# belinghy/SteppingStone

Measured on AMD Instinct MI355X. Metric: env-steps/sec (batched random-action rollout), higher is better.
Workload: dtype f32; 1 GPU; Walker3DStepperEnv-v0, 4096 envs per MI355X, curriculum 0 (flat terrain), on-device Philox U(-1,1) actions, auto-reset on; envs_total=4096, parallelism=env-shard x1, ranks=1, steps_per_launch=1000, prewarm_steps=256

## Files before the change

steppingstone_amd/csrc/ss_kernels.hpp:

```cpp
#pragma once
#include <cstdlib>

#include "ss_dynamics.hpp"
#include "../../include/steppingstone.h"

namespace ss {

enum { F_POS = 0, F_QUAT = 3, F_VEL = 7, F_Q = 13, F_QD = 34, F_POT = 55, F_ZINIT = 56, F_EPRET = 57, F_NNDR = 58,
       F_STONE = 59, F_HEAD = 59 + 24, F_EPRET_LO = 59 + 30, NF = 59 + 30 + 1 };
enum { I_N = 0, I_COUNT = 1, I_ELAPSED = 2, I_RNG = 3, I_FLAGS = 4, I_PROV = 5, NI = 6 };
constexpr int kNumStones = 20;
constexpr int kNumSubsteps = 4;
constexpr float kDeg = 0.017453292519943295f;

struct Knobs {
  const float* prob;
  int per_env_prob;
  int curriculum;
  float power;
  int auto_reset;
};

struct Params {
  float* fstate;
// ... 48 lines not shown
  philox4x32_10(ctr, 0u, P.env_offset + ((uint32_t)e & P.id_mask), 0u, P.seed_lo, P.seed_hi, out);
  ctr += 1u;
}

SSD int sample_cell(const Params& P, const Knobs& K, int e, float u) {
  float cdf = 0.f;
  int last = 0, pick = -1;
  const float* pr = K.per_env_prob ? K.prob + e : K.prob;
  const int stride = K.per_env_prob ? P.npad : 1;
#pragma unroll 1
  for (int k = 0; k < SS_NCELL; ++k) {
    float pk = pr[(size_t)k * stride];
    if (pk > 0.f) last = k;
    cdf += pk;
    if (pick < 0 && u < cdf) pick = k;
  }
  return pick < 0 ? last : pick;
}

SSD void place_stone(float px, float py, float pz, float dr, float cp, float sp, float cph, float sph, float out_p[3]) {
  float planar = dr * cp;
  out_p[0] = px + planar * cph;
  out_p[1] = py + planar * sph;
  out_p[2] = pz + dr * sp;
}
SSD float draw_stone(const Params& P, const Knobs& K, int e, uint32_t& ctr, int k, float out_p[3], float out_n[3],
                     float out_t[2], float out_h[2], bool store = true) {
  uint32_t r[4];
  env_block(P, e, ctr, r);
  int cell = sample_cell(P, K, e, u01(r[0]));
  float ratio = (float)K.curriculum / 5.0f;
  float dr = 0.65f + u01(r[1]) * (0.6f * ratio);
  float tilt = 15.0f * kDeg * ratio;
  float xt = (2.f * u01(r[2]) - 1.f) * tilt, yt = (2.f * u01(r[3]) - 1.f) * tilt;
  float yaw = yaw_sample(cell / SS_GRID), pitch = pitch_sample(cell % SS_GRID);
  const size_t np = (size_t)P.npad;
  float* T = P.terrain + e;
  int prov = P.istate[e + I_PROV * np];
  const bool prev_stored = k - 1 < prov;
  float px = prev_stored ? T[((k - 1) * 6 + 0) * np] : 0.75f * (float)(k - 1);
  float py = prev_stored ? T[((k - 1) * 6 + 1) * np] : 0.f, pz = prev_stored ? T[((k - 1) * 6 + 2) * np] : 0.f;
  float phi = (prev_stored ? T[((k - 1) * 6 + 3) * np] : 0.f) + yaw;
  float sp, cp, sph, cph;
  sincosf(pitch, &sp, &cp);
  sincosf(phi, &sph, &cph);
  place_stone(px, py, pz, dr, cp, sp, cph, sph, out_p);
  out_t[0] = xt; out_t[1] = yt;
  out_h[0] = cph; out_h[1] = sph;
  stone_normal(phi, xt, yt, out_n);
  if (store) {
#pragma unroll 1
    for (int j = prov; j < k; ++j) {
      T[(j * 6 + 0) * np] = 0.75f * (float)j;
#pragma unroll
      for (int i = 1; i < 6; ++i) T[(j * 6 + i) * np] = 0.f;
    }
    T[(k * 6 + 0) * np] = out_p[0]; T[(k * 6 + 1) * np] = out_p[1]; T[(k * 6 + 2) * np] = out_p[2];
    T[(k * 6 + 3) * np] = phi; T[(k * 6 + 4) * np] = xt; T[(k * 6 + 5) * np] = yt;
    if (prov < k + 1) P.istate[e + I_PROV * np] = k + 1;
  }
  return dr;
}

SSD float planar_dist(const float a[3], const float b[3]) {
  float dx = a[0] - b[0], dy = a[1] - b[1];
  return sqrtf(dx * dx + dy * dy);
}

SSD void quat_roll_pitch_cs(const float q[4], float& roll, float& pitch, float& cy, float& sy) {
  float w = q[0], x = q[1], y = q[2], z = q[3];
  roll = atan2f(2.f * (w * x + y * z), 1.f - 2.f * (x * x + y * y));
  pitch = asinf(fminf(fmaxf(2.f * (w * y - z * x), -1.f), 1.f));
  float A = 1.f - 2.f * (y * y + z * z), B = 2.f * (w * z + x * y);
  float n2 = A * A + B * B;
  float inv = SS_RSQRT(fmaxf(n2, 1e-30f));
  cy = n2 > 1e-30f ? A * inv : 1.f;
  sy = n2 > 1e-30f ? B * inv : 0.f;
}

SSD void target_features(const float pos[3], float cy, float sy, const float sp[3], const float tilt[2], float o[5]) {
  float dx = sp[0] - pos[0], dy = sp[1] - pos[1], dz = sp[2] - pos[2];
  o[0] = dy * cy - dx * sy; o[1] = dx * cy + dy * sy; o[2] = dz; o[3] = tilt[0]; o[4] = tilt[1];
}

SSD float clip5(float x) { return fminf(fmaxf(x, -5.f), 5.f); }
SSD float obs_angle(float ps, float q, float mid, float span) { return clip5(2.f * (ps * q - ps * mid) / span); }
SSD float obs_rate(float ps, float qd) { return clip5(0.1f * (ps * qd)); }

template <class Model>
SSD void write_obs(const Dyn& s, float z_init, int flags, const Cache& c, float* obs) {
  float roll, pitch, sy, cy;
  quat_roll_pitch_cs(s.quat, roll, pitch, cy, sy);
  float R[3][3];
  quat_rot(s.quat, R);
  float vw[3];
#pragma unroll
  for (int r = 0; r < 3; ++r) vw[r] = R[r][0] * s.v0.v[0] + R[r][1] * s.v0.v[1] + R[r][2] * s.v0.v[2];
  obs[0] = clip5(s.pos[2] - z_init);
  obs[1] = clip5(cy * vw[0] + sy * vw[1]);
  obs[2] = clip5(-sy * vw[0] + cy * vw[1]);
  obs[3] = clip5(vw[2]);
  obs[4] = clip5(roll);
  obs[5] = clip5(pitch);
  static_for<0, NJ>([&](auto Jc) {
    constexpr int j = decltype(Jc)::value;
    constexpr float mid = 0.5f * (Model::lo[j] + Model::hi[j]);
    constexpr float span = Model::hi[j] - Model::lo[j];
    constexpr float ps = (float)kPolicySign[j];
    obs[6 + j] = obs_angle(ps, s.q[j], mid, span);
    obs[27 + j] = obs_rate(ps, s.qd[j]);
  });
  obs[48] = (flags & 1) ? 1.f : 0.f;
  obs[49] = (flags & 2) ? 1.f : 0.f;
  float t[5];
  target_features(s.pos, cy, sy, c.p[1], c.tilt[1], t);
#pragma unroll
  for (int i = 0; i < 5; ++i) obs[50 + i] = t[i];
  target_features(s.pos, cy, sy, c.p[2], c.tilt[2], t);
#pragma unroll
  for (int i = 0; i < 5; ++i) obs[55 + i] = t[i];
}

SSD void load_dyn(const Params& P, int e, Dyn& s) {
  const float* F = P.fstate + e;
  const size_t np = (size_t)P.npad;
#pragma unroll
  for (int i = 0; i < 3; ++i) s.pos[i] = F[(F_POS + i) * np];
#pragma unroll
  for (int i = 0; i < 4; ++i) s.quat[i] = F[(F_QUAT + i) * np];
#pragma unroll
  for (int i = 0; i < 3; ++i) { s.v0.w[i] = F[(F_VEL + i) * np]; s.v0.v[i] = F[(F_VEL + 3 + i) * np]; }
#pragma unroll
  for (int j = 0; j < NJ; ++j) { s.q[j] = F[(F_Q + j) * np]; s.qd[j] = F[(F_QD + j) * np]; }
}
SSD void store_dyn(const Params& P, int e, const Dyn& s) {
  float* F = P.fstate + e;
  const size_t np = (size_t)P.npad;
#pragma unroll
  for (int i = 0; i < 3; ++i) F[(F_POS + i) * np] = s.pos[i];
#pragma unroll
  for (int i = 0; i < 4; ++i) F[(F_QUAT + i) * np] = s.quat[i];
#pragma unroll
  for (int i = 0; i < 3; ++i) { F[(F_VEL + i) * np] = s.v0.w[i]; F[(F_VEL + 3 + i) * np] = s.v0.v[i]; }
#pragma unroll
  for (int j = 0; j < NJ; ++j) { F[(F_Q + j) * np] = s.q[j]; F[(F_QD + j) * np] = s.qd[j]; }
}
SSD void load_cache(const Params& P, int e, Cache& c) {
  const float* F = P.fstate + e;
  const size_t np = (size_t)P.npad;
#pragma unroll
  for (int sl = 0; sl < 3; ++sl) {
#pragma unroll
    for (int i = 0; i < 3; ++i) { c.p[sl][i] = F[(F_STONE + sl * 8 + i) * np]; c.nrm[sl][i] = F[(F_STONE + sl * 8 + 3 + i) * np]; }
    c.tilt[sl][0] = F[(F_STONE + sl * 8 + 6) * np];
    c.tilt[sl][1] = F[(F_STONE + sl * 8 + 7) * np];
  }
}
SSD void store_cache(const Params& P, int e, const Cache& c) {
  float* F = P.fstate + e;
  const size_t np = (size_t)P.npad;
#pragma unroll
  for (int sl = 0; sl < 3; ++sl) {
#pragma unroll
    for (int i = 0; i < 3; ++i) { F[(F_STONE + sl * 8 + i) * np] = c.p[sl][i]; F[(F_STONE + sl * 8 + 3 + i) * np] = c.nrm[sl][i]; }
    F[(F_STONE + sl * 8 + 6) * np] = c.tilt[sl][0];
    F[(F_STONE + sl * 8 + 7) * np] = c.tilt[sl][1];
  }
}
SSD void store_headings(const Params& P, int e, const float (&h)[3][2]) {
  float* F = P.fstate + e;
  const size_t np = (size_t)P.npad;
#pragma unroll
  for (int sl = 0; sl < 3; ++sl) { F[(F_HEAD + sl * 2) * np] = h[sl][0]; F[(F_HEAD + sl * 2 + 1) * np] = h[sl][1]; }
}
SSD void cache_from_terrain(const Params& P, int e, int n, Cache& c, float (&hd)[3][2]) {
  const size_t np = (size_t)P.npad;
  const float* T = P.terrain + e;
  int idx[3] = {n - 1 < 0 ? 0 : n - 1, n, n + 1 > kNumStones - 1 ? kNumStones - 1 : n + 1};
#pragma unroll
  for (int sl = 0; sl < 3; ++sl) {
    int k = idx[sl];
#pragma unroll
    for (int i = 0; i < 3; ++i) c.p[sl][i] = T[(k * 6 + i) * np];
    float phi = T[(k * 6 + 3) * np], xt = T[(k * 6 + 4) * np], yt = T[(k * 6 + 5) * np];
    c.tilt[sl][0] = xt; c.tilt[sl][1] = yt;
    stone_normal(phi, xt, yt, c.nrm[sl]);
    sincosf(phi, &hd[sl][1], &hd[sl][0]);
  }
}

SSD void flat_path(Stones& c) {
#pragma unroll
  for (int sl = 0; sl < 3; ++sl) {
    c.p[sl][0] = 0.75f * (float)sl; c.p[sl][1] = 0.f; c.p[sl][2] = 0.f;
    c.nrm[sl][0] = 0.f; c.nrm[sl][1] = 0.f; c.nrm[sl][2] = 1.f;
    c.tilt[sl][0] = 0.f; c.tilt[sl][1] = 0.f;
  }
}
template <class Model, int GJ>
SSD float reset_angle(const uint32_t (&r)[6][4]) {
  constexpr float q0 = Model::q0[GJ], lo = Model::lo[GJ] + 0.02f, hi = Model::hi[GJ] - 0.02f;
  float q = q0 + 0.05f * (2.f * u01(r[GJ / 4][GJ % 4]) - 1.f);
  return fminf(fmaxf(q, lo), hi);
}

template <class Model>
SSD void env_reset(const Params& P, int e, Dyn& s, Cache& c, uint32_t& ctr, float& pot, float& z_init, float& nn_dr) {
  const size_t np = (size_t)P.npad;
  P.istate[e + I_PROV * np] = 0;
  flat_path(c);
  s.pos[0] = 0.f; s.pos[1] = 0.f; s.pos[2] = Model::stand_height + 0.01f;
  s.quat[0] = 1.f; s.quat[1] = s.quat[2] = s.quat[3] = 0.f;
#pragma unroll
  for (int i = 0; i < 3; ++i) { s.v0.w[i] = 0.f; s.v0.v[i] = 0.f; }
  uint32_t r[6][4];
#pragma unroll
  for (int b = 0; b < 6; ++b) env_block(P, e, ctr, r[b]);
  static_for<0, NJ>([&](auto Jc) {
    constexpr int j = decltype(Jc)::value;
    s.q[j] = reset_angle<Model, j>(r);
    s.qd[j] = 0.f;
  });
  z_init = s.pos[2];
  nn_dr = 0.75f;
  pot = -planar_dist(c.p[1], s.pos) / kDt;
}

constexpr int kMaxPeers = 8;
struct PeerTable {
  float* dst[kMaxPeers];
  uint32_t* flag[kMaxPeers];
  uint32_t* done_counter;
  int count;
  int rank;
  int n_local;
};

struct StepIO {
  const float* act;
  float* obs;
  float* rew;
  uint8_t* done;
  ss_info* info;
  uint64_t t;
  float* packed;
  int nsteps;
  const PeerTable* peers;
  uint32_t flag_value;
  long long packed_step_stride;
};

SSD void put_base(const Lds& L, float m, const float pos[3], const float quat[4], const float w[3], const float v[3]) {
  L.s(S_POS + 0) = pos[0]; L.s(S_POS + 1) = m * pos[1]; L.s(S_POS + 2) = pos[2];
  L.s(S_QUAT + 0) = quat[0]; L.s(S_QUAT + 1) = m * quat[1]; L.s(S_QUAT + 2) = quat[2]; L.s(S_QUAT + 3) = m * quat[3];
  L.s(S_VW + 0) = m * w[0]; L.s(S_VW + 1) = w[1]; L.s(S_VW + 2) = m * w[2];
  L.s(S_VV + 0) = v[0]; L.s(S_VV + 1) = m * v[1]; L.s(S_VV + 2) = v[2];
}
SSD void get_base(const Lds& L, float m, float pos[3], float quat[4], SV& v0) {
  pos[0] = L.s(S_POS); pos[1] = m * L.s(S_POS + 1); pos[2] = L.s(S_POS + 2);
  quat[0] = L.s(S_QUAT); quat[1] = m * L.s(S_QUAT + 1); quat[2] = L.s(S_QUAT + 2); quat[3] = m * L.s(S_QUAT + 3);
  v0 = SV{{m * L.s(S_VW), L.s(S_VW + 1), m * L.s(S_VW + 2)}, {L.s(S_VV), m * L.s(S_VV + 1), L.s(S_VV + 2)}};
}
SSD void put_joints(const Lds& L, float m, const float (&q)[NH], const float (&qd)[NH]) {
  static_for<0, NH>([&](auto Kc) {
    constexpr int k = decltype(Kc)::value, jr = kHalf[k];
    const float sg = mirror_sign(jr, m);
    L.s(S_Q + k) = sg * q[k];
    L.s(S_QD + k) = sg * qd[k];
  });
}
SSD void get_joints(const Lds& L, float m, float (&q)[NH], float (&qd)[NH]) {
  static_for<0, NH>([&](auto Kc) {
    constexpr int k = decltype(Kc)::value, jr = kHalf[k];
    const float sg = mirror_sign(jr, m);
    q[k] = sg * L.s(S_Q + k);
    qd[k] = sg * L.s(S_QD + k);
  });
}

struct StepOut {
  float pos[3], quat[4];
  SV v0;
  float qt[NH], qdt[NH];
  float r, z_init, roll, pitch, cyaw, syaw;
  int d, flags, do_reset;
// ... 115 lines not shown
    if constexpr (!ROLLOUT) {
      if (io.peers) {
        constexpr int kPack = SS_OBS_DIM + 2;
        const PeerTable* T = io.peers;
        const int G = T->count;
        const size_t row0 = (size_t)T->rank * (size_t)T->n_local + (size_t)env0;
#pragma unroll 1
        for (int p = 0; p < G; ++p) copy_block(T->dst[p] + row0 * kPack, nvalid * kPack);
        __threadfence_system();
        if (lane == 0) {
          const uint32_t prev = atomicAdd(T->done_counter, 1u);
          if ((prev + 1u) % gridDim.x == 0u) {
            __threadfence_system();
            for (int p = 0; p < G; ++p)
              __hip_atomic_store(T->flag[p] + T->rank, io.flag_value, __ATOMIC_RELEASE, __HIP_MEMORY_SCOPE_SYSTEM);
          }
        }
      }
    }
#endif
  }
#undef SS_OBS
}

constexpr bool out_offload(int helpers, bool rollout) { return rollout && helpers >= 3; }
constexpr int kHandOut = kHandDet, kHandOut2 = kHandFloats;
static_assert(kHandOut2 + 2 <= kHandSlots * 4, "hand-off region");
#if !defined(SS_HOST_HARNESS)
template <class Model, bool ROLLOUT>
__device__ __forceinline__ void emit_from_handoff(const Params& P, const StepIO& io, const Lds& L, int lane, int lane_global, int kstep,
                                                  float* lds) {
  const int e_raw = lane_global >> 1, side = lane_global & 1;
  const bool valid = e_raw < P.n;
  const int e = valid ? e_raw : P.n - 1;
  const float m = side ? -1.f : 1.f;
  StepOut o;
  get_base(L, m, o.pos, o.quat, o.v0);
  get_joints(L, m, o.qt, o.qdt);
  o.r = L.hs(kHandOut + 0);
  o.z_init = L.hs(kHandOut + 1);
  {
    const float w = L.hs(kHandOut + 2), w2 = xchg(w);
    o.inf.ep_ret = side ? w2 : w;
    o.inf.ep_ret_lo = side ? w : w2;
  }
  const int bits = __builtin_bit_cast(int, L.hs(kHandOut2 + 0));
  o.d = bits & 1;
  o.inf.bad_transition = (bits >> 1) & 1;
  o.inf.update_terrain = (bits >> 2) & 1;
  o.do_reset = (bits >> 3) & 1;
  o.flags = (bits >> 4) & 3;
  o.inf.steps_reached = (bits >> 8) & 31;
  o.inf.ep_len = (float)((bits >> 16) & 0xffff);
#pragma unroll
  for (int i = 0; i < 5; ++i) { o.tgt[0][i] = L.hs(kHandOut + 3 + i); o.tgt[1][i] = L.hs(kHandOut + 8 + i); }
  quat_roll_pitch_cs(o.quat, o.roll, o.pitch, o.cyaw, o.syaw);
  emit_outputs<Model, ROLLOUT>(P, io, o, e, side, valid, lane, lane_global, kstep, lds);
}
#endif

template <class Write>
SSD void random_actions_half(const Params& P, int e, int side, float m, uint32_t tt, Write&& write) {
  uint32_t ra[6][4];
#pragma unroll
  for (int b = 0; b < 6; ++b) philox4x32_10(6u * tt + b, 1u, P.env_offset + ((uint32_t)e & P.id_mask), 0u, P.seed_lo, P.seed_hi, ra[b]);
  static_for<0, NH>([&](auto Kc) {
    constexpr int k = decltype(Kc)::value, jr = kHalf[k];
    constexpr int jl = left_twin(jr);
    const float sg = action_lane_sign(jr, m);
    const uint32_t bits = side ? ra[jl / 4][jl % 4] : ra[jr / 4][jr % 4];
    write(k, sg * (2.f * u01(bits) - 1.f));
  });
}

template <class Model, bool RANDOM_ACT, int HELPERS = 0, bool ROLLOUT = false>
SSD void step_env(const Params& P, const StepIO& io, int lane_global, int lane, float* lds) {
  static_assert(!ROLLOUT || RANDOM_ACT, "a multi-step launch draws its actions on the device");
  constexpr bool kOffload =
#if defined(__HIP_DEVICE_COMPILE__)
      out_offload(HELPERS, ROLLOUT);
#else
      false;
#endif
  const int e_raw = lane_global >> 1, side = lane_global & 1;
  const bool valid = e_raw < P.n;
  int e = valid ? e_raw : P.n - 1;
  const size_t np = (size_t)P.npad;
  const float m = side ? -1.f : 1.f;
  const Lds L{lds, lane};
  const float* F = P.fstate + e;

  {
    Cache c0;
    load_cache(P, e, c0);
    float h0[3][2];
#pragma unroll
    for (int sl = 0; sl < 3; ++sl) { h0[sl][0] = F[(F_HEAD + sl * 2) * np]; h0[sl][1] = F[(F_HEAD + sl * 2 + 1) * np]; }
#pragma unroll
    for (int sl = 0; sl < 3; ++sl) {
      L.s(S_STP + sl * 3 + 0) = c0.p[sl][0]; L.s(S_STP + sl * 3 + 1) = m * c0.p[sl][1]; L.s(S_STP + sl * 3 + 2) = c0.p[sl][2];
      L.s(S_STN + sl * 3 + 0) = c0.nrm[sl][0]; L.s(S_STN + sl * 3 + 1) = m * c0.nrm[sl][1]; L.s(S_STN + sl * 3 + 2) = c0.nrm[sl][2];
      L.q2(kLdsHead + sl) = make_float2(h0[sl][0], m * h0[sl][1]);
    }
  }

  float gin[13], qin[NH], qdin[NH];
#pragma unroll
  for (int i = 0; i < 3; ++i) gin[i] = F[(F_POS + i) * np];
#pragma unroll
  for (int i = 0; i < 4; ++i) gin[3 + i] = F[(F_QUAT + i) * np];
#pragma unroll
  for (int i = 0; i < 6; ++i) gin[7 + i] = F[(F_VEL + i) * np];
  static_for<0, NH>([&](auto Kc) {
    constexpr int k = decltype(Kc)::value, jr = kHalf[k];
    constexpr int jl = left_twin(jr);
    const int gj = side ? jl : jr;
    qin[k] = F[(F_Q + gj) * np];
    qdin[k] = F[(F_QD + gj) * np];
  });
  float ain[NH];
  if constexpr (!RANDOM_ACT) {
    static_for<0, NH>([&](auto Kc) {
      constexpr int k = decltype(Kc)::value, jr = kHalf[k];
      constexpr int jl = left_twin(jr);
      ain[k] = io.act[(size_t)e * NJ + (side ? jl : jr)];
    });
  }
  put_base(L, m, gin, gin + 3, gin + 7, gin + 10);
  put_joints(L, m, qin, qdin);

  const int nsteps = ROLLOUT ? io.nsteps : 1;
#pragma unroll 1
  for (int kstep = 0; kstep < nsteps; ++kstep) {
  SS_FUZZ(0x60u);
  if constexpr (RANDOM_ACT) {
    bool drawn = false;
    if constexpr (ROLLOUT && HELPERS > 1) {
      if (kstep > 0) {
        float a[NH];
#pragma unroll
        for (int k = 0; k < NH; ++k) a[k] = L.hs(kHandAct + k);
#pragma unroll
        for (int k = 0; k < NH; ++k) L.s(S_ACT + k) = a[k];
        drawn = true;
      }
    }
    if (!drawn) random_actions_half(P, e, side, m, (uint32_t)io.t + (uint32_t)kstep, [&](int k, float a) { L.s(S_ACT + k) = a; });
  } else {
    static_for<0, NH>([&](auto Kc) {
      constexpr int k = decltype(Kc)::value, jr = kHalf[k];
      const float sg = action_lane_sign(jr, m);
      const float x = ain[k];
      float a = fminf(fmaxf(x, -1.f), 1.f);
      a = (x != x) ? x : a;
      L.s(S_ACT + k) = sg * a;
    });
  }

  const float power = P.knobs->power;
  FootReport fr;
#if defined(SS_PROFILE_PHASES) && defined(__HIP_DEVICE_COMPILE__)
  Prof prof;
#pragma unroll
  for (int i = 0; i < 16; ++i) prof.t[i] = 0;
  prof.last = (uint32_t)__builtin_amdgcn_s_memtime();
#endif
  Warm wm;
  warm_clear(wm);
  if constexpr (warm_in_lds(HELPERS)) L.s(S_WKEY) = 0.f;
#pragma unroll 1
  for (int k = 0; k < kNumSubsteps; ++k) substep<Model, HELPERS>(SS_PROF_ARG power, fr, L, wm);
  SS_FUZZ(0x61u);
  SS_PROF(12);
  SS_MEMBAR();
  SS_OPAQUE(e);
  F = P.fstate + e;
  const Knobs K = *P.knobs;
  Cache c;
  load_cache(P, e, c);
  float pot_prev = F[F_POT * np], z_init = F[F_ZINIT * np];
  float ep_ret = F[F_EPRET * np], ep_lo = F[F_EPRET_LO * np], nn_dr = F[F_NNDR * np];
  int n = P.istate[e + I_N * np], count = P.istate[e + I_COUNT * np], elapsed = P.istate[e + I_ELAPSED * np];
  uint32_t ctr = (uint32_t)P.istate[e + I_RNG * np];
  SS_PROFE(1);

  float pos[3], quat[4];
  SV v0;
  get_base(L, m, pos, quat, v0);
  elapsed += 1;
  const float my_sole[3] = {fr.sole[0], m * fr.sole[1], fr.sole[2]};
  float ot_sole[3];
#pragma unroll
  for (int i = 0; i < 3; ++i) ot_sole[i] = xchg(my_sole[i]);
  const int ot_contact = xchg_i(fr.contact), ot_target = xchg_i(fr.on_target);
  float sole[2][3];
#pragma unroll
  for (int i = 0; i < 3; ++i) { sole[0][i] = side ? ot_sole[i] : my_sole[i]; sole[1][i] = side ? my_sole[i] : ot_sole[i]; }
  int flags = side ? (ot_contact | (fr.contact << 1)) : (fr.contact | (ot_contact << 1));
  const int on_target = fr.on_target | ot_target;
  SS_PROFE(2);
  float accv = 0.f, e_sum = 0.f, a2 = 0.f;
  int at_limit = 0;
  static_for<0, NH>([&](auto Kc) {
    constexpr int k = decltype(Kc)::value, jr = kHalf[k];
    constexpr float mid = 0.5f * (Model::lo[jr] + Model::hi[jr]);
    constexpr float span = Model::hi[jr] - Model::lo[jr];
    const float q = L.s(S_Q + k), qd = L.s(S_QD + k), a = L.s(S_ACT + k);
    const bool mine = (jr >= 3) || (side == 0);
    accv += q + qd;
    if (mine) {
      e_sum += fabsf(a * (0.1f * qd));
      a2 += a * a;
      if (fabsf(2.f * (q - mid) / span) > 0.99f) at_limit += 1;
    }
  });
  accv += pos[0] + pos[1] + pos[2] + quat[0] + quat[1] + quat[2] + quat[3];
#pragma unroll
  for (int i = 0; i < 3; ++i) accv += v0.w[i] + v0.v[i];
  e_sum += xchg(e_sum);
  a2 += xchg(a2);
  at_limit += xchg_i(at_limit);
  const bool finite = finite_bits(accv) && (xchg_i(finite_bits(accv) ? 1 : 0) != 0);
  SS_PROFE(3);

  float target_old[3] = {c.p[1][0], c.p[1][1], c.p[1][2]};
  float step_bonus = 0.f;
  int advanced = 0;
  float hd[3][2] = {{1.f, 0.f}, {1.f, 0.f}, {1.f, 0.f}};
  if (on_target != 0) {
    count += 1;
    if (count == 1) {
      float d0 = planar_dist(sole[0], target_old), d1 = planar_dist(sole[1], target_old);
      step_bonus = 50.f * expf(-fminf(d0, d1) / 0.25f);
    }
    if (count >= 2 && n < kNumStones - 1) {
      n += 1;
      count = 0;
      advanced = 1;
#pragma unroll
      for (int i = 0; i < 3; ++i) {
        c.p[0][i] = c.p[1][i]; c.nrm[0][i] = c.nrm[1][i];
        c.p[1][i] = c.p[2][i]; c.nrm[1][i] = c.nrm[2][i];
      }
      c.tilt[0][0] = c.tilt[1][0]; c.tilt[0][1] = c.tilt[1][1];
      c.tilt[1][0] = c.tilt[2][0]; c.tilt[1][1] = c.tilt[2][1];
      const float2 h1 = L.q2(kLdsHead + 1), h2 = L.q2(kLdsHead + 2);
      hd[0][0] = h1.x; hd[0][1] = m * h1.y;
      hd[1][0] = h2.x; hd[1][1] = m * h2.y;
      hd[2][0] = h2.x; hd[2][1] = m * h2.y;
      if (n + 1 <= kNumStones - 1) nn_dr = draw_stone(P, K, e, ctr, n + 1, c.p[2], c.nrm[2], c.tilt[2], hd[2], valid && side == 0);
      L.q2(kLdsHead + 0) = h1;
      L.q2(kLdsHead + 1) = h2;
      L.q2(kLdsHead + 2) = make_float2(hd[2][0], m * hd[2][1]);
    }
  }
  float pot = -planar_dist(target_old, pos) / kDt;
  SS_PROFE(4);
  float progress = pot - pot_prev;
  pot_prev = advanced ? -planar_dist(c.p[1], pos) / kDt : pot;
  float target_bonus = (n == kNumStones - 1 && planar_dist(c.p[1], pos) < 0.15f) ? 2.f : 0.f;
  float zs = fminf(sole[0][2], sole[1][2]);
  float tall_bonus = (pos[2] - zs > 0.7f) ? 2.f : -1.f;
  float zlow = fminf(fminf(c.p[0][2], c.p[1][2]), c.p[2][2]);
  bool d = (tall_bonus < 0.f) || (pos[2] < zlow + 0.3f) || !finite;
  bool timeout = elapsed >= SS_MAX_EPISODE_STEPS;
  int bad = timeout ? 1 : 0;
  d = d || timeout;
  float roll, pitch, cyaw, syaw;
  quat_roll_pitch_cs(quat, roll, pitch, cyaw, syaw);
  float posture = 0.f;
  if (!(pitch > -0.2f && pitch < 0.4f)) posture += fabsf(pitch);
  if (!(roll > -0.4f && roll < 0.4f)) posture += fabsf(roll);
  float energy = (4.5f / NJ) * (e_sum / NJ) + (0.225f / NJ) * (a2 / NJ);
  float r = progress + step_bonus + target_bonus + tall_bonus - energy - posture - 0.1f * (float)at_limit;
  if (!finite || !finite_bits(r)) r = 0.f;
  SS_PROFE(5);
  {
    const float s = ep_ret + r, bb = s - ep_ret;
    const float err = (ep_ret - (s - bb)) + (r - bb);
    const float lo = ep_lo + err;
    ep_ret = s + lo;
    ep_lo = lo - (ep_ret - s);
  }
  ss_info inf;
  inf.ep_ret = ep_ret;
  inf.ep_ret_lo = ep_lo;
  inf.ep_len = (float)elapsed;
  inf.bad_transition = bad;
  inf.steps_reached = n;
  inf.update_terrain = advanced;
  const bool do_reset = d && K.auto_reset;
  SS_PROFE(6);
  uint32_t rr[6][4];
  if (do_reset) {
    if (valid && side == 0) P.istate[e + I_PROV * np] = 0;
    flat_path(c);
#pragma unroll
    for (int sl = 0; sl < 3; ++sl) {
      hd[sl][0] = 1.f; hd[sl][1] = 0.f;
      L.q2(kLdsHead + sl) = make_float2(1.f, 0.f);
    }
    pos[0] = 0.f; pos[1] = 0.f; pos[2] = Model::stand_height + 0.01f;
    quat[0] = 1.f; quat[1] = quat[2] = quat[3] = 0.f;
#pragma unroll
    for (int i = 0; i < 3; ++i) { v0.w[i] = 0.f; v0.v[i] = 0.f; }
    {
      uint32_t c3 = ctr + (side ? 3u : 0u), mine[3][4];
#pragma unroll
      for (int b = 0; b < 3; ++b) env_block(P, e, c3, mine[b]);
#pragma unroll
      for (int b = 0; b < 3; ++b)
#pragma unroll
        for (int i = 0; i < 4; ++i) {
          const uint32_t other = xchg_u32(mine[b][i]);
          rr[b][i] = side ? other : mine[b][i];
          rr[3 + b][i] = side ? mine[b][i] : other;
        }
      ctr += 6u;
    }
    z_init = pos[2];
    nn_dr = 0.75f;
    pot_prev = -planar_dist(c.p[1], pos) / kDt;
    n = 1; count = 0; elapsed = 0; flags = 0; ep_ret = 0.f; ep_lo = 0.f;
  }
  SS_PROFE(7);
  float qt[NH], qdt[NH];
  static_for<0, NH>([&](auto Kc) {
    constexpr int k = decltype(Kc)::value, jr = kHalf[k];
    constexpr int jl = left_twin(jr);
    const float sg = mirror_sign(jr, m);
    if (do_reset) {
      qt[k] = side ? reset_angle<Model, jl>(rr) : reset_angle<Model, jr>(rr);
      qdt[k] = 0.f;
    } else {
      qt[k] = sg * L.s(S_Q + k);
      qdt[k] = sg * L.s(S_QD + k);
    }
  });
  SS_PROFE(8);
  SS_FUZZ(0x62u);
  if constexpr (ROLLOUT) {
    if (do_reset) {
      put_base(L, m, pos, quat, v0.w, v0.v);
      put_joints(L, m, qt, qdt);
    }
    if (advanced || do_reset) {
#pragma unroll
      for (int sl = 0; sl < 3; ++sl) {
        L.s(S_STP + sl * 3 + 0) = c.p[sl][0]; L.s(S_STP + sl * 3 + 1) = m * c.p[sl][1]; L.s(S_STP + sl * 3 + 2) = c.p[sl][2];
        L.s(S_STN + sl * 3 + 0) = c.nrm[sl][0]; L.s(S_STN + sl * 3 + 1) = m * c.nrm[sl][1]; L.s(S_STN + sl * 3 + 2) = c.nrm[sl][2];
      }
    }
  }
  if constexpr (kOffload) {
    L.hs(kHandOut + 0) = r;
    L.hs(kHandOut + 1) = z_init;
    L.hs(kHandOut + 2) = side ? inf.ep_ret_lo : inf.ep_ret;
    const int bits = (d ? 1 : 0) | (inf.bad_transition << 1) | (inf.update_terrain << 2) | ((do_reset ? 1 : 0) << 3) | (flags << 4) |
                     (inf.steps_reached << 8) | ((int)inf.ep_len << 16);
    L.hs(kHandOut2 + 0) = __builtin_bit_cast(float, bits);
#pragma unroll
    for (int i = 0; i < 3; ++i) { L.hs(kHandOut + 3 + i) = c.p[1][i]; L.hs(kHandOut + 8 + i) = c.p[2][i]; }
#pragma unroll
    for (int i = 0; i < 2; ++i) { L.hs(kHandOut + 6 + i) = c.tilt[1][i]; L.hs(kHandOut + 11 + i) = c.tilt[2][i]; }
  } else {
    StepOut o;
#pragma unroll
    for (int i = 0; i < 3; ++i) o.pos[i] = pos[i];
#pragma unroll
    for (int i = 0; i < 4; ++i) o.quat[i] = quat[i];
    o.v0 = v0;
#pragma unroll
    for (int k = 0; k < NH; ++k) { o.qt[k] = qt[k]; o.qdt[k] = qdt[k]; }
    o.r = r; o.z_init = z_init; o.roll = roll; o.pitch = pitch; o.cyaw = cyaw; o.syaw = syaw;
    o.d = d ? 1 : 0; o.flags = flags; o.do_reset = do_reset ? 1 : 0;
#pragma unroll
    for (int i = 0; i < 3; ++i) { o.tgt[0][i] = c.p[1][i]; o.tgt[1][i] = c.p[2][i]; }
#pragma unroll
    for (int i = 0; i < 2; ++i) { o.tgt[0][3 + i] = c.tilt[1][i]; o.tgt[1][3 + i] = c.tilt[2][i]; }
    o.inf = inf;
    emit_outputs<Model, ROLLOUT>(P, io, o, e, side, valid, lane, lane_global, kstep, lds);
  }
  if (valid && side == 0) {
  SS_PROFE(9);
    float* Fo = P.fstate + e;
    if (advanced || do_reset) {
      store_cache(P, e, c);
      store_headings(P, e, hd);
    }
    Fo[F_POT * np] = pot_prev;
    Fo[F_ZINIT * np] = z_init;
    Fo[F_EPRET * np] = ep_ret;
    Fo[F_EPRET_LO * np] = ep_lo;
    Fo[F_NNDR * np] = nn_dr;
    P.istate[e + I_N * np] = n;
    P.istate[e + I_COUNT * np] = count;
    P.istate[e + I_ELAPSED * np] = elapsed;
    P.istate[e + I_RNG * np] = (int)ctr;
    P.istate[e + I_FLAGS * np] = flags;
  }
  SS_MEMBAR();
#if defined(SS_PROFILE_PHASES) && defined(__HIP_DEVICE_COMPILE__)
  SS_PROFE(10);
  SS_PROF(13);
  if (lane == 0 && P.prof)
    for (int i = 0; i < 16; ++i) atomicAdd(P.prof + i, (unsigned long long)prof.t[i]);
#endif
  }
#if defined(__HIP_DEVICE_COMPILE__)
  if constexpr (out_offload(HELPERS, ROLLOUT)) __syncthreads();
#endif
}

#ifndef SS_HOST_HARNESS
template <class Model, bool RANDOM_ACT>
__global__ __launch_bounds__(kWave, 1) void step_kernel(Params P, StepIO io) {
  __shared__ float4 lds4[kLdsSlots * kWave];
  step_env<Model, RANDOM_ACT>(P, io, blockIdx.x * kWave + threadIdx.x, threadIdx.x, reinterpret_cast<float*>(lds4));
}
template <class Model, bool RANDOM_ACT, int HELPERS>
__global__ __launch_bounds__(kWave * (1 + HELPERS), 1) void step_kernel_helped(Params P, StepIO io) {
  __shared__ float4 lds4[(kLdsSlots + hand_slots(HELPERS)) * kWave];
  const int wave = __builtin_amdgcn_readfirstlane(threadIdx.x >> 6), lane = threadIdx.x & (kWave - 1);
  float* lds = reinterpret_cast<float*>(lds4);
  SS_FUZZ(0x70u + wave);
  if (wave == 0) {
    step_env<Model, RANDOM_ACT, HELPERS>(P, io, blockIdx.x * kWave + lane, lane, lds);
// ... 139 lines not shown
```

steppingstone_amd/csrc/ss_math.hpp:

```cpp
#pragma once
#include <hip/hip_runtime.h>

#include <type_traits>

#include "ss_model_tables.hpp"

#define SSD __host__ __device__ __forceinline__

#if defined(__HIP_DEVICE_COMPILE__)
#define SS_OPAQUE(x) asm volatile("" : "+v"(x))
#define SS_RSQRT(x) rsqrtf(x)
static __device__ __forceinline__ float ss_rcp(float x) {
  float r = __builtin_amdgcn_rcpf(x);
  return __builtin_fmaf(__builtin_fmaf(-x, r, 1.0f), r, r);
}
#define SS_RCP(x) ss_rcp(x)
#define SS_UMULHI(a, b) __umulhi((a), (b))
#define SS_F2U(x) __float_as_uint(x)
#else
#include <cmath>
#include <cstring>
float ss_host_xchg(float x);
void ss_host_wave_sync();
static inline float ss_host_rsqrt(float x) { return 1.0f / sqrtf(x); }
static inline unsigned ss_host_umulhi(unsigned a, unsigned b) { return (unsigned)(((unsigned long long)a * b) >> 32); }
static inline unsigned ss_host_f2u(float x) { unsigned u; std::memcpy(&u, &x, 4); return u; }
#define SS_OPAQUE(x) asm volatile("" : "+r"(x))
#define SS_RSQRT(x) ss_host_rsqrt(x)
#define SS_RCP(x) (1.0f / (x))
#define SS_UMULHI(a, b) ss_host_umulhi((a), (b))
#define SS_F2U(x) ss_host_f2u(x)
#endif
#define SS_ACC(o, k, x)                       \
  do {                                        \
    if constexpr ((k) != 0.0f) (o) += (k) * (x); \
  } while (0)

namespace ss {

constexpr int NJ = 21;
constexpr int NB = 22;
constexpr int RFOOT = 8;
constexpr int LFOOT = 13;

template <int I, int N, class F>
SSD void static_for(F&& f) {
  if constexpr (I < N) {
    f(std::integral_constant<int, I>{});
    static_for<I + 1, N>(f);
  }
}
template <int I, int LO, class F>
SSD void static_rfor(F&& f) {
  if constexpr (I >= LO) {
    f(std::integral_constant<int, I>{});
    static_rfor<I - 1, LO>(f);
  }
}

constexpr int first_child(int b) {
  int r = -1;
  for (int j = 0; j < NJ; ++j)
    if (kParent[j] == b) r = j + 1;
  return r;
}
constexpr bool on_leg_path(int b) {
  return (b >= 1 && b <= 13);
}

struct SV {
  float w[3];
  float v[3];
};

struct Sym3 {
  float m[6];
  template <int I, int J>
  SSD float& at() {
    if constexpr (I == J) return m[I];
    else if constexpr (I + J == 1) return m[3];
    else if constexpr (I + J == 2) return m[4];
    else return m[5];
  }
  template <int I, int J>
  SSD float get() const {
    if constexpr (I == J) return m[I];
    else if constexpr (I + J == 1) return m[3];
    else if constexpr (I + J == 2) return m[4];
    else return m[5];
  }
};

struct ABI {
  Sym3 A;
  float B[3][3];
  Sym3 C;
};

SSD void cross(const float a[3], const float b[3], float o[3]) {
  float x = a[1] * b[2] - a[2] * b[1], y = a[2] * b[0] - a[0] * b[2], z = a[0] * b[1] - a[1] * b[0];
  o[0] = x; o[1] = y; o[2] = z;
}
SSD float dot3(const float a[3], const float b[3]) { return a[0] * b[0] + a[1] * b[1] + a[2] * b[2]; }
SSD float dot6(const SV& a, const SV& b) { return dot3(a.w, b.w) + dot3(a.v, b.v); }

template <int AX>
SSD void rot(float c, float s, const float v[3], float o[3]) {
  constexpr int i = (AX + 1) % 3, j = (AX + 2) % 3;
  float vi = v[i], vj = v[j];
  o[AX] = v[AX];
  o[i] = c * vi - s * vj;
  o[j] = s * vi + c * vj;
}
// ... 182 lines not shown
  cross(v.w, f, p.v);
  return p;
}

SSD void abi_dense(const ABI& I, float M[6][6]) {
  const Sym3 &A = I.A, &C = I.C;
  float Af[3][3] = {{A.m[0], A.m[3], A.m[4]}, {A.m[3], A.m[1], A.m[5]}, {A.m[4], A.m[5], A.m[2]}};
  float Cf[3][3] = {{C.m[0], C.m[3], C.m[4]}, {C.m[3], C.m[1], C.m[5]}, {C.m[4], C.m[5], C.m[2]}};
#pragma unroll
  for (int i = 0; i < 3; ++i)
#pragma unroll
    for (int j = 0; j < 3; ++j) {
      M[i][j] = Af[i][j];
      M[i][j + 3] = I.B[i][j];
      M[i + 3][j] = I.B[j][i];
      M[i + 3][j + 3] = Cf[i][j];
    }
}

struct Chol6 {
  float l[15];
  float di[6];
  template <int I, int J>
  SSD float& at() { return l[I * (I - 1) / 2 + J]; }
  template <int I, int J>
  SSD float get() const { return l[I * (I - 1) / 2 + J]; }
};

SSD Chol6 chol6(const float M[6][6]) {
  Chol6 L;
  static_for<0, 6>([&](auto Ic) {
    constexpr int i = decltype(Ic)::value;
    static_for<0, i + 1>([&](auto Jc) {
      constexpr int j = decltype(Jc)::value;
      float s = M[i][j];
      static_for<0, j>([&](auto Kc) {
        constexpr int k = decltype(Kc)::value;
        if constexpr (i == j) s -= L.template get<i, k>() * L.template get<i, k>();
        else s -= L.template get<i, k>() * L.template get<j, k>();
      });
      if constexpr (i == j) L.di[i] = SS_RSQRT(s);
      else L.template at<i, j>() = s * L.di[j];
    });
  });
  return L;
}
SSD SV chol6_solve_neg(const Chol6& L, const SV& b) {
  float y[6] = {-b.w[0], -b.w[1], -b.w[2], -b.v[0], -b.v[1], -b.v[2]};
  static_for<0, 6>([&](auto Ic) {
    constexpr int i = decltype(Ic)::value;
    float s = y[i];
    static_for<0, i>([&](auto Kc) {
      constexpr int k = decltype(Kc)::value;
      s -= L.template get<i, k>() * y[k];
    });
    y[i] = s * L.di[i];
  });
  static_rfor<5, 0>([&](auto Ic) {
    constexpr int i = decltype(Ic)::value;
    float s = y[i];
    static_for<i + 1, 6>([&](auto Kc) {
      constexpr int k = decltype(Kc)::value;
      s -= L.template get<k, i>() * y[k];
    });
    y[i] = s * L.di[i];
  });
  SV x;
  x.w[0] = y[0]; x.w[1] = y[1]; x.w[2] = y[2]; x.v[0] = y[3]; x.v[1] = y[4]; x.v[2] = y[5];
  return x;
}

SSD void quat_rot(const float q[4], float R[3][3]) {
  float w = q[0], x = q[1], y = q[2], z = q[3];
  R[0][0] = 1.f - 2.f * (y * y + z * z); R[0][1] = 2.f * (x * y - w * z); R[0][2] = 2.f * (x * z + w * y);
  R[1][0] = 2.f * (x * y + w * z); R[1][1] = 1.f - 2.f * (x * x + z * z); R[1][2] = 2.f * (y * z - w * x);
  R[2][0] = 2.f * (x * z - w * y); R[2][1] = 2.f * (y * z + w * x); R[2][2] = 1.f - 2.f * (x * x + y * y);
}

SSD bool finite_bits(float x) { return (SS_F2U(x) & 0x7f800000u) != 0x7f800000u; }

SSD void philox4x32_10(uint32_t c0, uint32_t c1, uint32_t c2, uint32_t c3, uint32_t k0, uint32_t k1, uint32_t out[4]) {
#pragma unroll
  for (int r = 0; r < 10; ++r) {
    uint32_t h0 = SS_UMULHI(0xD2511F53u, c0), l0 = 0xD2511F53u * c0;
    uint32_t h1 = SS_UMULHI(0xCD9E8D57u, c2), l1 = 0xCD9E8D57u * c2;
    uint32_t n0 = h1 ^ c1 ^ k0, n2 = h0 ^ c3 ^ k1;
    c0 = n0; c1 = l1; c2 = n2; c3 = l0;
    k0 += 0x9E3779B9u; k1 += 0xBB67AE85u;
  }
  out[0] = c0; out[1] = c1; out[2] = c2; out[3] = c3;
}
SSD float u01(uint32_t x) { return (float)(x >> 8) * 5.9604644775390625e-08f; }

}
```

Baseline: 90.19 million env-steps/s.

## Branchless reward terms, division-free limit test, lean reset path and 64-bit Philox

Several micro-optimizations in the step kernel. The joint-limit check now compares against a per-joint threshold computed at compile time instead of dividing by the span, and energy and posture accumulation become select-based instead of branches. In the offload rollout path, reset joint angles are computed and written straight to LDS only inside the reset branch, which drops the per-step qt/qdt staging. Philox now takes its high and low halves from a single 64-bit product instead of umulhi plus a separate multiply. These are small instruction-count savings; the threshold search has to reproduce the original rounding exactly, or limit counts will drift.

```diff
diff --git a/steppingstone_amd/csrc/ss_kernels.hpp b/steppingstone_amd/csrc/ss_kernels.hpp
--- a/steppingstone_amd/csrc/ss_kernels.hpp
+++ b/steppingstone_amd/csrc/ss_kernels.hpp
@@ -154,6 +154,16 @@
   float dx = sp[0] - pos[0], dy = sp[1] - pos[1], dz = sp[2] - pos[2];
   o[0] = dy * cy - dx * sy; o[1] = dx * cy + dy * sy; o[2] = dz; o[3] = tilt[0]; o[4] = tilt[1];
 }
+
+constexpr float ulp_step(float x, int d) { return __builtin_bit_cast(float, __builtin_bit_cast(uint32_t, x) + (uint32_t)d); }
+constexpr float limit_threshold(float span) {
+  float t = 0.99f * span;
+  while (t / span > 0.99f) t = ulp_step(t, -1);
+  while (!(t / span > 0.99f)) t = ulp_step(t, 1);
+  return t;
+}
+template <class Model>
+constexpr float joint_limit_threshold(int j) { return limit_threshold(Model::hi[j] - Model::lo[j]); }
 
 SSD float clip5(float x) { return fminf(fmaxf(x, -5.f), 5.f); }
 SSD float obs_angle(float ps, float q, float mid, float span) { return clip5(2.f * (ps * q - ps * mid) / span); }
@@ -273,6 +283,16 @@
 SSD float reset_angle(const uint32_t (&r)[6][4]) {
   constexpr float q0 = Model::q0[GJ], lo = Model::lo[GJ] + 0.02f, hi = Model::hi[GJ] - 0.02f;
   float q = q0 + 0.05f * (2.f * u01(r[GJ / 4][GJ % 4]) - 1.f);
+  return fminf(fmaxf(q, lo), hi);
+}
+
+template <class Model, int JR>
+SSD float reset_angle_half(const uint32_t (&r)[6][4], int side) {
+  constexpr int JL = left_twin(JR);
+  const uint32_t w = side ? r[JL / 4][JL % 4] : r[JR / 4][JR % 4];
+  const float q0 = side ? Model::q0[JL] : Model::q0[JR];
+  const float lo = side ? Model::lo[JL] + 0.02f : Model::lo[JR] + 0.02f, hi = side ? Model::hi[JL] - 0.02f : Model::hi[JR] - 0.02f;
+  float q = q0 + 0.05f * (2.f * u01(w) - 1.f);
   return fminf(fmaxf(q, lo), hi);
 }
 
@@ -554,6 +574,7 @@
 #else
       false;
 #endif
+  constexpr bool kResetOnly = ROLLOUT && kOffload;
   const int e_raw = lane_global >> 1, side = lane_global & 1;
   const bool valid = e_raw < P.n;
   int e = valid ? e_raw : P.n - 1;
@@ -676,15 +697,13 @@
   static_for<0, NH>([&](auto Kc) {
     constexpr int k = decltype(Kc)::value, jr = kHalf[k];
     constexpr float mid = 0.5f * (Model::lo[jr] + Model::hi[jr]);
-    constexpr float span = Model::hi[jr] - Model::lo[jr];
+    constexpr float T = joint_limit_threshold<Model>(jr);
     const float q = L.s(S_Q + k), qd = L.s(S_QD + k), a = L.s(S_ACT + k);
     const bool mine = (jr >= 3) || (side == 0);
     accv += q + qd;
-    if (mine) {
-      e_sum += fabsf(a * (0.1f * qd));
-      a2 += a * a;
-      if (fabsf(2.f * (q - mid) / span) > 0.99f) at_limit += 1;
-    }
+    e_sum += mine ? fabsf(a * (0.1f * qd)) : 0.f;
+    a2 += mine ? a * a : 0.f;
+    at_limit += (mine && fabsf(2.f * (q - mid)) >= T) ? 1 : 0;
   });
   accv += pos[0] + pos[1] + pos[2] + quat[0] + quat[1] + quat[2] + quat[3];
 #pragma unroll
@@ -740,9 +759,8 @@
   d = d || timeout;
   float roll, pitch, cyaw, syaw;
   quat_roll_pitch_cs(quat, roll, pitch, cyaw, syaw);
-  float posture = 0.f;
-  if (!(pitch > -0.2f && pitch < 0.4f)) posture += fabsf(pitch);
-  if (!(roll > -0.4f && roll < 0.4f)) posture += fabsf(roll);
+  float posture = (!(pitch > -0.2f && pitch < 0.4f)) ? fabsf(pitch) : 0.f;
+  posture += (!(roll > -0.4f && roll < 0.4f)) ? fabsf(roll) : 0.f;
   float energy = (4.5f / NJ) * (e_sum / NJ) + (0.225f / NJ) * (a2 / NJ);
   float r = progress + step_bonus + target_bonus + tall_bonus - energy - posture - 0.1f * (float)at_limit;
   if (!finite || !finite_bits(r)) r = 0.f;
@@ -794,27 +812,41 @@
     nn_dr = 0.75f;
     pot_prev = -planar_dist(c.p[1], pos) / kDt;
     n = 1; count = 0; elapsed = 0; flags = 0; ep_ret = 0.f; ep_lo = 0.f;
+    if constexpr (kResetOnly) {
+      float qr[NH], qdr[NH];
+      static_for<0, NH>([&](auto Kc) {
+        constexpr int k = decltype(Kc)::value, jr = kHalf[k];
+        qr[k] = reset_angle_half<Model, jr>(rr, side);
+        qdr[k] = 0.f;
+      });
+      put_base(L, m, pos, quat, v0.w, v0.v);
+      put_joints(L, m, qr, qdr);
+    }
   }
   SS_PROFE(7);
-  float qt[NH], qdt[NH];
-  static_for<0, NH>([&](auto Kc) {
-    constexpr int k = decltype(Kc)::value, jr = kHalf[k];
-    constexpr int jl = left_twin(jr);
-    const float sg = mirror_sign(jr, m);
-    if (do_reset) {
-      qt[k] = side ? reset_angle<Model, jl>(rr) : reset_angle<Model, jr>(rr);
-      qdt[k] = 0.f;
-    } else {
-      qt[k] = sg * L.s(S_Q + k);
-      qdt[k] = sg * L.s(S_QD + k);
-    }
-  });
+  [[maybe_unused]] float qt[NH], qdt[NH];
+  if constexpr (!kResetOnly) {
+    static_for<0, NH>([&](auto Kc) {
+      constexpr int k = decltype(Kc)::value, jr = kHalf[k];
+      constexpr int jl = left_twin(jr);
+      const float sg = mirror_sign(jr, m);
+      if (do_reset) {
+        qt[k] = side ? reset_angle<Model, jl>(rr) : reset_angle<Model, jr>(rr);
+        qdt[k] = 0.f;
+      } else {
+        qt[k] = sg * L.s(S_Q + k);
+        qdt[k] = sg * L.s(S_QD + k);
+      }
+    });
+  }
   SS_PROFE(8);
   SS_FUZZ(0x62u);
   if constexpr (ROLLOUT) {
-    if (do_reset) {
-      put_base(L, m, pos, quat, v0.w, v0.v);
-      put_joints(L, m, qt, qdt);
+    if constexpr (!kResetOnly) {
+      if (do_reset) {
+        put_base(L, m, pos, quat, v0.w, v0.v);
+        put_joints(L, m, qt, qdt);
+      }
     }
     if (advanced || do_reset) {
 #pragma unroll
diff --git a/steppingstone_amd/csrc/ss_math.hpp b/steppingstone_amd/csrc/ss_math.hpp
--- a/steppingstone_amd/csrc/ss_math.hpp
+++ b/steppingstone_amd/csrc/ss_math.hpp
@@ -15,7 +15,6 @@
   return __builtin_fmaf(__builtin_fmaf(-x, r, 1.0f), r, r);
 }
 #define SS_RCP(x) ss_rcp(x)
-#define SS_UMULHI(a, b) __umulhi((a), (b))
 #define SS_F2U(x) __float_as_uint(x)
 #else
 #include <cmath>
@@ -23,12 +22,10 @@
 float ss_host_xchg(float x);
 void ss_host_wave_sync();
 static inline float ss_host_rsqrt(float x) { return 1.0f / sqrtf(x); }
-static inline unsigned ss_host_umulhi(unsigned a, unsigned b) { return (unsigned)(((unsigned long long)a * b) >> 32); }
 static inline unsigned ss_host_f2u(float x) { unsigned u; std::memcpy(&u, &x, 4); return u; }
 #define SS_OPAQUE(x) asm volatile("" : "+r"(x))
 #define SS_RSQRT(x) ss_host_rsqrt(x)
 #define SS_RCP(x) (1.0f / (x))
-#define SS_UMULHI(a, b) ss_host_umulhi((a), (b))
 #define SS_F2U(x) ss_host_f2u(x)
 #endif
 #define SS_ACC(o, k, x)                       \
@@ -377,8 +374,9 @@
 SSD void philox4x32_10(uint32_t c0, uint32_t c1, uint32_t c2, uint32_t c3, uint32_t k0, uint32_t k1, uint32_t out[4]) {
 #pragma unroll
   for (int r = 0; r < 10; ++r) {
-    uint32_t h0 = SS_UMULHI(0xD2511F53u, c0), l0 = 0xD2511F53u * c0;
-    uint32_t h1 = SS_UMULHI(0xCD9E8D57u, c2), l1 = 0xCD9E8D57u * c2;
+    const uint64_t p0 = (uint64_t)0xD2511F53u * c0, p1 = (uint64_t)0xCD9E8D57u * c2;
+    uint32_t h0 = (uint32_t)(p0 >> 32), l0 = (uint32_t)p0;
+    uint32_t h1 = (uint32_t)(p1 >> 32), l1 = (uint32_t)p1;
     uint32_t n0 = h1 ^ c1 ^ k0, n2 = h0 ^ c3 ^ k1;
     c0 = n0; c1 = l1; c2 = n2; c3 = l0;
     k0 += 0x9E3779B9u; k1 += 0xBB67AE85u;
```

Result: no change. 90.41 million env-steps/s (median of 5 runs) (+0.2%).
